# Cyame/glpk.js

Hardware: AMD Instinct MI355X
Metric: simplex pivots/s (dual, C3 dense 4096x16384 fp64) (higher is better)
Workload: dtype f64; 1 GPU; C3 dense random LP m=4096 n=16384 (BASELINE.json configs[2]); step = glp_simplex dual with it_lim=100 continuing from the previous basis; m=4096, n=16384, parallelism=replicas x1

## Files before the change

### glpk.js_amd/csrc/gk_dual.hip

```cpp
#include "gk_device.h"
#include <hip/hip_ext.h>
#include <algorithm>
#include <cstdlib>
#include <stdexcept>

namespace gk {

template <int NRHS, typename XF>
__device__ __forceinline__ void lgemv_tile(const double *__restrict__ M, size_t ld, int rows,
                                           const int *__restrict__ list, int t0, int t1, int r, XF xf,
                                           double *__restrict__ o)
{
    if (r >= rows) return;
    double a0 = 0.0, a1 = 0.0, b0 = 0.0, b1 = 0.0;
    int t = t0;
    for (; t + 4 <= t1; t += 4) {
        int c[4];
        double xa[4], xb[4];
        bool any = false;
#pragma unroll
        for (int u = 0; u < 4; ++u) {
            c[u] = list[t + u];
            xf(t + u, c[u], xa[u], xb[u]);
            any = any || xa[u] != 0.0 || xb[u] != 0.0;
// ... 185 lines not shown
    if (t < 0.0) t = 0.0;
    if (!(t <= tmax)) return false;
    e.k1 = t; e.k2 = fabs(alfa); e.idx = j + 1; e.aux = k;
    return true;
}

__device__ __forceinline__ Cand pass1_slot(const SpxDev &d, const RatioCtx &x, int idx)
{
    const int m = d.m, n = d.n;
    Cand best = no_cand(DBL_MAX);
    if (idx < n) {
        const int pos = d.bind[m + idx];
        if (pos > m) {
            const int j = pos - m - 1;
            Cand e;
            if (pass1_cand(x, d.trow[j], d.cbar[j], d.stat[j], j, m + idx + 1, e) && better<1>(e, best)) best = e;
        }
    }
    if (idx < m) {
        const int pos = d.bind[idx];
        if (pos > m) {
            const int j = pos - m - 1;
            Cand e;
            if (pass1_cand(x, d.trow[j], d.cbar[j], d.stat[j], j, idx + 1, e) && better<1>(e, best)) best = e;
        }
    }
    return best;
}

struct TopState {
    int iter_left, refact, refct;
    double obj;
};

struct FinishIn {
    int pend, p, q, kp, kq, fxp, rclr, upd_cnt, it_cnt, npiv, rig;
    double delta;
    TopState t;
};

__device__ __forceinline__ FinishIn finish_load(const SpxDev &d)
{
    const DState *st = d.st;
    FinishIn f;
    const int pend = st->pend, iter_left = st->iter_left, rpend = st->refact_pending, upd_cnt = st->upd_cnt,
              upd_lim = st->upd_lim, pricing = st->pricing, refct = st->refct, phase = st->phase;
    const double obj = st->obj, cqo = st->cbar_q_old, zeta = st->zeta, delta = st->delta, pivot = st->pivot;
    f.p = st->p; f.q = st->q; f.kp = st->kp; f.kq = st->kq;
    f.fxp = st->fxp; f.rclr = st->rclr; f.it_cnt = st->it_cnt; f.npiv = st->npiv;
    f.rig = st->rigorous;
    f.pend = pend;
    f.upd_cnt = upd_cnt;
    f.delta = delta;
    f.t.iter_left = iter_left - pend;
    f.t.refact = (rpend != 0) | ((pend != 0) & (upd_cnt + 1 >= upd_lim));
    f.t.refct = ((pend != 0) & (pricing == PT_PSE) & (refct > 0)) ? refct - 1 : refct;
    const double dobj = (cqo / zeta) * (delta / pivot);
    f.t.obj = ((pend != 0) & (phase == 2)) ? obj + dobj : obj;
    return f;
}

__device__ TopState finish_apply(const SpxDev &d, const FinishIn &f, bool tail_sync)
{
    DState *st = d.st;
    const int m = d.m;
    __syncthreads();
// ... 12 lines not shown
            st->binv_fresh = 0;
            st->cbar_fresh = 0;
            st->refact_pending = f.t.refact;
            st->it_cnt = f.it_cnt + 1;
            st->npiv = f.npiv + 1;
            st->iter_left = f.t.iter_left;
            if (f.rig > 0) st->rigorous = f.rig - 1;
            st->refct = f.t.refct;
            st->pend = 0;
        }
    }
    if (tail_sync) __syncthreads();
    return f.t;
}

__device__ __forceinline__ void finish_arrays(const SpxDev &d, const FinishIn &f)
{
    const int m = d.m;
    __syncthreads();
    if (f.pend) {
        if (threadIdx.x == 0) {
            d.head[f.p - 1] = f.kq;
            d.head[m + f.q - 1] = f.kp;
            d.bind[f.kq - 1] = f.p;
            d.bind[f.kp - 1] = m + f.q;
            d.stat[f.q - 1] = f.fxp ? NS : (f.delta > 0.0 ? NL : NU);
        } else if (threadIdx.x == 64) {
            if (f.rclr) d.refsp[f.kp - 1] = 0;
        }
    }
    __syncthreads();
}

__device__ __forceinline__ void finish_scalars(const SpxDev &d, const FinishIn &f, bool refsp_reset)
{
    DState *st = d.st;
    if (f.pend) {
        st->obj = f.t.obj;
        st->upd_cnt = f.upd_cnt + 1;
        st->binv_fresh = 0;
        st->cbar_fresh = 0;
        st->refact_pending = f.t.refact;
        st->it_cnt = f.it_cnt + 1;
        st->npiv = f.npiv + 1;
        st->iter_left = f.t.iter_left;
        if (f.rig > 0) st->rigorous = f.rig - 1;
        st->refct = f.t.refct;
        st->pend = 0;
    }
    if (refsp_reset) st->refct = 1000;
}

__device__ TopState dual_finish_block(const SpxDev &d, bool tail_sync)
{
    return finish_apply(d, finish_load(d), tail_sync);
}

__global__ void k_dual_finish(SpxDev d)
{
    (void)dual_finish_block(d, true);
}

__device__ __forceinline__ Cand chuzr_cand_v(int i, int k, int t, double lb, double ub, double bb, double g,
                                             double tol_bnd)
{
    double ri = 0.0;
// ... 82 lines not shown
    const double zeta = st->zeta, obj_ll = st->obj_ll, obj_ul = st->obj_ul;
    if (stop) return;
    const TopState ts = finish_apply(d, fin, false);
    if (ts.iter_left <= 0 || ts.refact) {
        if (threadIdx.x == 0) st->stop = ts.refact ? ST_REFACT : ST_BATCH;
        return;
    }
    if (pricing == PT_PSE && ts.refct == 0) {
        __syncthreads();
        reset_refsp_dev(d, 1);
        for (int l = threadIdx.x; l < n; l += blockDim.x) d.wpos[l] = -1;
        if (threadIdx.x == 0) st->nwl = 0;
        __syncthreads();
    }
    if (phase == 1) {
        if (!dinf) {
            if (threadIdx.x == 0) st->stop = ST_PHASE;
            return;
        }
    } else {
        const double z = zeta, obj = ts.obj;
        const bool hit = (z < 0.0 && obj_ll > -DBL_MAX && obj <= obj_ll) ||
                         (z > 0.0 && obj_ul < +DBL_MAX && obj >= obj_ul);
        if (hit) {
            if (threadIdx.x == 0) st->stop = ST_OBJLIM;
            return;
        }
    }
    const Cand best = wave_best<0>(c);
    if (best.idx == 0) {
        if (threadIdx.x == 0) { st->p = 0; st->stop = ST_P0; }
        return;
    }
    const int p = best.idx, kp = best.aux;
    if (rowpath == 3) {
        if (threadIdx.x == 0) {
            st->p = p;
            st->kp = kp;
            st->delta = best.k2;
            st->trow_max_bits = 0ull;
            st->ns = 0;
            st->dinf = 0;
        }
        return;
    }
    if (!rowpath) {
        for (int l = threadIdx.x; l < m; l += blockDim.x) d.rho[l] = 0.0;
        __syncthreads();
    }
    const double *brow = d.Binv + (p - 1);
    const size_t ldb = (size_t)d.ldb;
    double v[RPT];
#pragma unroll
    for (int u = 0; u < RPT; ++u) {
        const int t = threadIdx.x + u * TOP_WG;
        v[u] = (t < nr) ? brow[(size_t)cl[u] * ldb] : 0.0;
    }
#pragma unroll
    for (int u = 0; u < RPT; ++u) {
        const int t = threadIdx.x + u * TOP_WG;
        if (t < nr) {
            if (!rowpath) d.rho[cl[u]] = v[u];
            d.rho_idx[t] = cl[u];
            d.rho_val[t] = v[u];
        }
    }
    for (int t = threadIdx.x + RPT * TOP_WG; t < nr; t += blockDim.x) {
        const int cc = d.rlist[t];
        const double vv = brow[(size_t)cc * ldb];
        if (!rowpath) d.rho[cc] = vv;
        d.rho_idx[t] = cc;
        d.rho_val[t] = vv;
    }
    if (threadIdx.x == 0) {
        int ns = nr;
        if (kp <= m) {
            if (!rowpath) d.rho[kp - 1] = 1.0;
            d.rho_idx[nr] = kp - 1;
            d.rho_val[nr] = 1.0;
            ns++;
        }
        st->p = p;
        st->kp = kp;
        st->delta = best.k2;
        st->trow_max_bits = 0ull;
        st->ns = ns;
        st->dinf = 0;
    }
}

template <int PANEL>
__global__ void __launch_bounds__(256) k_dual_top_grid(SpxDev d, int pcap, int page_max)
{
    const TraceScope trace_(d, 0);
    DState *st = d.st;
    const int m = d.m, n = d.n;
    const int lane = threadIdx.x & 63;
    const bool lead = (blockIdx.x == 0);
    const int stop = st->stop;
    const FinishIn fin = finish_load(d);
    const int pricing = st->pricing, phase = st->phase, dinf = st->dinf, nr = st->nr;
    const double zeta = st->zeta, obj_ll = st->obj_ll, obj_ul = st->obj_ul;
    const int gm = 4 * ((m + 255) / 256);
    Cand cc = no_cand(0.0);
    for (int b = lane; b < gm; b += 64) {
        const Cand e = cand_chuzr(d)[b];
        if (better<0>(e, cc)) cc = e;
    }
    const int i = blockIdx.x * 256 + threadIdx.x;
    const int rp = (i < m) ? d.rpos[i] : -1;
    const int cl = (i < nr) ? d.rlist[i] : 0;
    if (stop) return;
    const TopState ts = fin.t;
    int why = ST_RUN;
    if (ts.iter_left <= 0 || ts.refact) why = ts.refact ? ST_REFACT : ST_BATCH;
    else if (phase == 1 && !dinf) why = ST_PHASE;
    else if (phase != 1 && ((zeta < 0.0 && obj_ll > -DBL_MAX && ts.obj <= obj_ll) ||
                            (zeta > 0.0 && obj_ul < +DBL_MAX && ts.obj >= obj_ul)))
        why = ST_OBJLIM;
    const Cand best = wave_best<0>(cc);
    if (why == ST_RUN && best.idx == 0) why = ST_P0;
    gate_arrive(st);
    if (why != ST_RUN) {
        if (lead) {
            if (threadIdx.x == 0) gate_wait(st);
            finish_arrays(d, fin);
            if (threadIdx.x == 0) {
                finish_scalars(d, fin, false);
                if (why == ST_P0) st->p = 0;
                st->stop = why;
            }
        }
        return;
    }
    const bool reset = pricing == PT_PSE && ts.refct == 0;
    if (lead) {
        if (threadIdx.x == 0) gate_wait(st);
        finish_arrays(d, fin);
        if (reset) {
            reset_refsp_dev(d, 1, false);
            for (int l = threadIdx.x; l < n; l += blockDim.x) d.wpos[l] = -1;
            if (threadIdx.x == 0) st->nwl = 0;
        }
        if (threadIdx.x == 0) finish_scalars(d, fin, reset);
    }
    const int p = best.idx, kp = best.aux;
    const double *brow = d.Binv + (p - 1);
    const size_t ldb = (size_t)d.ldb;
    const double vr = (i < m && rp >= 0) ? brow[(size_t)i * ldb] : 0.0;
    const double vl = (i < nr) ? brow[(size_t)cl * ldb] : 0.0;
    if (i < m) d.rho[i] = (rp >= 0) ? vr : (i == kp - 1 ? 1.0 : 0.0);
    if (i < nr) {
        d.rho_idx[i] = cl;
        d.rho_val[i] = vl;
// ... 218 lines not shown
    int c0[NP];
#pragma unroll
    for (int u = 0; u < NP; ++u) c0[u] = d.rlist[min(w + u * nw, m - 1)];
    int pos1 = d.bind[m + min(idx, n - 1)];
    int pos2 = d.bind[min(idx, m - 1)];
    const double *__restrict__ col = d.A.AT + min(idx, n - 1);
    const size_t ldt = (size_t)d.A.ldt;
    double a0[NP];
#pragma unroll
    for (int u = 0; u < NP; ++u) a0[u] = col[(size_t)min(max(c0[u], 0), m - 1) * ldt];
    Cand cc = no_cand(0.0);
#pragma unroll
    for (int u = 0; u < 4; ++u)
        if (lane + 64 * u < gm && better<0>(ce[u], cc)) cc = ce[u];
    for (int b = lane + 256; b < gm; b += 64) {
        const Cand e = cand_chuzr(d)[b];
        if (better<0>(e, cc)) cc = e;
    }
#pragma unroll
    for (int u = 0; u < NP; ++u) c0[u] = (w + u * nw < nr_cap) ? c0[u] : 0;
    if (w != 0 || idx >= n) pos1 = 0;
    if (w != 0 || idx >= m) pos2 = 0;
    if (stop) return;
    if (d.tslots && lead && threadIdx.x == 0) st->tk_start = wall_clock64();
    const TopState ts = fin.t;
    int why = ST_RUN;
    if (ts.iter_left <= 0 || ts.refact) why = ts.refact ? ST_REFACT : ST_BATCH;
    else if (phase == 1 && !dinf) why = ST_PHASE;
    else if (phase != 1 && ((zeta < 0.0 && obj_ll > -DBL_MAX && ts.obj <= obj_ll) ||
                            (zeta > 0.0 && obj_ul < +DBL_MAX && ts.obj >= obj_ul)))
        why = ST_OBJLIM;
    const Cand best = wave_best<0>(cc);
    if (why == ST_RUN && best.idx == 0) why = ST_P0;
    const bool reset = (why == ST_RUN && pricing == PT_PSE && ts.refct == 0);
    if (why != ST_RUN) {
        gate_arrive(st);
        if (lead) {
            if (threadIdx.x == 0) gate_wait(st);
            finish_arrays(d, fin);
            if (threadIdx.x == 0) {
                finish_scalars(d, fin, false);
                if (why == ST_P0) st->p = 0;
                st->stop = why;
            }
        }
        return;
    }
    if (lead) {
        finish_arrays(d, fin);
        if (reset) {
            reset_refsp_dev(d, 1, false);
            for (int l = threadIdx.x; l < n; l += blockDim.x) d.wpos[l] = -1;
            if (threadIdx.x == 0) st->nwl = 0;
        }
    }
    const int p = best.idx, kp = best.aux;
    const int ns = nr + (kp <= m ? 1 : 0);
    auto bind_new = [&](int k1, int v) {
        if (!fin.pend) return v;
        if (k1 == fin.kq) return fin.p;
        if (k1 == fin.kp) return m + fin.q;
        return v;
    };
    if (w == 0 && idx < n) pos1 = bind_new(m + idx + 1, pos1);
    if (w == 0 && idx < m) pos2 = bind_new(idx + 1, pos2);
    const int j1 = (pos1 > m) ? pos1 - m - 1 : -1;
    const int j2 = (pos2 > m) ? pos2 - m - 1 : -1;
    const double *__restrict__ brow = d.Binv + (p - 1);
    const size_t ldb = (size_t)d.ldb;
    double v0[NP];
#pragma unroll
    for (int u = 0; u < NP; ++u) {
        const int t = w + u * nw;
        int c = c0[u];
        double av = a0[u];
        if (t == nr) {
            c = kp - 1;
            av = col[(size_t)min(max(c, 0), m - 1) * ldt];
        }
        const int ca = min(max(c, 0), m - 1);
        const double bv = brow[(size_t)ca * ldb];
        v0[u] = (t < nr) ? bv : 1.0;
        a0[u] = (t < ns) ? av : 0.0;
        c0[u] = c;
    }
    const signed char stq = fin.fxp ? NS : (fin.delta > 0.0 ? NL : NU);
    int s1 = 0, s2 = 0;
    double cb1 = 0.0, cb2 = 0.0, rho2 = 0.0;
    bool ref1 = false, ref2 = false;
    if (w == 0) {
        const int j1c = max(j1, 0), j2c = max(j2, 0);
        const int l1 = d.stat[j1c], l2 = d.stat[j2c];
        const double c1 = d.cbar[j1c], c2 = d.cbar[j2c];
        const double r2 = brow[(size_t)min(idx, m - 1) * ldb];
        const int f1 = d.refsp[m + min(idx, n - 1)], f2 = d.refsp[min(idx, m - 1)];
        if (j1 >= 0) {
            s1 = (fin.pend && j1 == fin.q - 1) ? stq : l1;
            cb1 = c1;
            if (pse && !reset) ref1 = f1 != 0 && !(fin.pend && fin.rclr && m + idx + 1 == fin.kp);
        }
        if (j2 >= 0) {
            s2 = (fin.pend && j2 == fin.q - 1) ? stq : l2;
            cb2 = c2;
            rho2 = r2;
            if (pse && !reset) ref2 = f2 != 0 && !(fin.pend && fin.rclr && idx + 1 == fin.kp);
        }
    }
    double acc = 0.0;
#pragma unroll
    for (int u = 0; u < NP; ++u)
        if (w + u * nw < ns) acc += v0[u] * a0[u];
    if (lead && lane == 0) {
#pragma unroll
        for (int u = 0; u < NP; ++u) {
            const int t = w + u * nw;
            if (t < ns) {
                d.rho_idx[t] = c0[u];
                d.rho_val[t] = v0[u];
            }
        }
    }
    TPH(1, 0);
    {
        int t = w + NP * nw;
        for (; t < ns; t += 4 * nw) {
            int c[4];
            double v[4], a[4];
#pragma unroll
            for (int u = 0; u < 4; ++u) {
                const int tt = t + u * nw;
                c[u] = (tt < nr) ? d.rlist[tt] : kp - 1;
            }
#pragma unroll
            for (int u = 0; u < 4; ++u) {
                const int tt = t + u * nw;
                v[u] = (tt < nr) ? brow[(size_t)c[u] * ldb] : 1.0;
                a[u] = (tt < ns) ? col[(size_t)c[u] * ldt] : 0.0;
            }
#pragma unroll
            for (int u = 0; u < 4; ++u)
// ... 85 lines not shown
    constexpr int CU = 8;
    int beg = 0, end = 0;
    if (idx < n) {
        beg = d.A.cptr[idx];
        end = d.A.cptr[idx + 1];
    }
    int ci[CU];
    double cv[CU];
#pragma unroll
    for (int u = 0; u < CU; ++u) {
        const bool ok = beg + u < end;
        ci[u] = ok ? d.A.cind[beg + u] : 0;
        cv[u] = ok ? d.A.cval[beg + u] : 0.0;
    }
    constexpr int PU = 4;
    const int tpub = blockIdx.x * blockDim.x + threadIdx.x, npub = gridDim.x * blockDim.x;
    int cpub[PU];
#pragma unroll
    for (int u = 0; u < PU; ++u) {
        const int t = tpub + u * npub;
        cpub[u] = (t < nr_cap) ? d.rlist[t] : 0;
    }
    if (stop) return;
    if (d.tslots && lead && threadIdx.x == 0) st->tk_start = wall_clock64();
    const TopState ts = fin.t;
    int why = ST_RUN;
    if (ts.iter_left <= 0 || ts.refact) why = ts.refact ? ST_REFACT : ST_BATCH;
    else if (phase == 1 && !dinf) why = ST_PHASE;
    else if (phase != 1 && ((zeta < 0.0 && obj_ll > -DBL_MAX && ts.obj <= obj_ll) ||
                            (zeta > 0.0 && obj_ul < +DBL_MAX && ts.obj >= obj_ul)))
        why = ST_OBJLIM;
    const Cand best = wave_best<0>(cc);
    if (why == ST_RUN && best.idx == 0) why = ST_P0;
    const bool reset = (why == ST_RUN && pricing == PT_PSE && ts.refct == 0);
    gate_arrive(st);
    if (why != ST_RUN) {
        if (lead) {
            if (threadIdx.x == 0) gate_wait(st);
            finish_arrays(d, fin);
            if (threadIdx.x == 0) {
                finish_scalars(d, fin, false);
                if (why == ST_P0) st->p = 0;
                st->stop = why;
            }
        }
        return;
    }
    if (lead) {
        finish_arrays(d, fin);
        if (reset) {
            reset_refsp_dev(d, 1, false);
            for (int l = threadIdx.x; l < n; l += blockDim.x) d.wpos[l] = -1;
            if (threadIdx.x == 0) st->nwl = 0;
        }
    }
    const int p = best.idx, kp = best.aux;
    const int ns = nr + (kp <= m ? 1 : 0);
    auto bind_new = [&](int k1, int v) {
        if (!fin.pend) return v;
        if (k1 == fin.kq) return fin.p;
        if (k1 == fin.kp) return m + fin.q;
        return v;
    };
    if (idx < n) pos1 = bind_new(m + idx + 1, pos1);
    if (idx < m) pos2 = bind_new(idx + 1, pos2);
    const int j1 = (pos1 > m) ? pos1 - m - 1 : -1;
// ... 176 lines not shown
    }
    if ((int)blockIdx.x >= gn) {
        const int b = blockIdx.x - gn;
        const int tile = b % tiles_m, split = b / tiles_m, splits = (gridDim.x - gn) / tiles_m;
        const int cnt = st->nwl;
        if (stop) return;
        const int lps = (cnt + splits - 1) / splits;
        const int t0 = split * lps, t1 = min(cnt, t0 + lps);
        const int r = (tile * 256 + threadIdx.x) * 2;
        const double *wc = d.wcol;
        lgemv_tile<1>(d.A.A, (size_t)d.A.lda, m, d.wlist, t0, t1, r,
                      [&](int, int c, double &xa, double &xb) { xa = wc[c]; xb = 0.0; },
                      d.awpart + (size_t)split * m);
        __shared__ int last;
        __threadfence();
        __syncthreads();
        if (threadIdx.x == 0) last = (atomicAdd(&d.awcnt[tile], 1) == splits - 1);
        __syncthreads();
        if (!last) return;
        __threadfence();
        for (int rr = r; rr < min(r + 2, m); ++rr) {
            double acc = 0.0;
            for (int sp = 0; sp < splits; ++sp) acc += d.awpart[(size_t)sp * m + rr];
            d.work[rr] = d.ys[rr] - acc;
        }
        if (threadIdx.x == 0) d.awcnt[tile] = 0;
        return;
    }
    const int lane = threadIdx.x & 63;
    const bool stamps = d.tslots != nullptr;
    const unsigned long long t_entry = (stamps && rowpath && blockIdx.x == 0 && threadIdx.x == 0) ? wall_clock64() : 0ull;
    RatioIn rin = ratio_in(st);
    if (rowpath == 1) rin.delta = st->ob_delta;
    const int j = blockIdx.x * blockDim.x + threadIdx.x;
    const int jc = min(j, n - 1);
    double trj = d.trow[jc], cbj = d.cbar[jc];
    int sj = d.stat[jc], kj = d.head[m + jc];
    const bool lead = (blockIdx.x == 0 && threadIdx.x < 64);
    constexpr int CPL = 8;
    const bool bsplit = ncb > CPL * 64;
    const int tb = bsplit ? (int)threadIdx.x : lane, tst = bsplit ? (int)blockDim.x : 64;
    Cand cl[CPL];
    double tv[CPL];
#pragma unroll
    for (int u = 0; u < CPL; ++u) {
        const int b = min(tb + u * tst, ncb - 1);
        cl[u] = cand_pass1(d)[b];
        tv[u] = tmax_part(d)[b];
    }
    unsigned long long e = 0, xp = 0, u0 = 0;
    double uticks = 0.0, un = 0.0;
    if (stamps && rowpath && lead) {
        u0 = st->tk_upd0;
        uticks = st->upd_ticks;
        un = st->upd_n;
        unsigned long long te[CPL], tx[4];
#pragma unroll
        for (int u = 0; u < CPL; ++u) te[u] = d.tslots[min(lane + u * 64, ncb - 1)];
#pragma unroll
        for (int u = 0; u < 4; ++u) tx[u] = d.xslots[min(lane + u * 64, max(nprev - 1, 0))];
#pragma unroll
        for (int u = 0; u < CPL; ++u) e = max(e, te[u]);
#pragma unroll
        for (int u = 0; u < 4; ++u) xp = max(xp, tx[u]);
        for (int b = lane + CPL * 64; b < ncb; b += 64) e = max(e, d.tslots[b]);
        for (int b = lane + 4 * 64; b < nprev; b += 64) xp = max(xp, d.xslots[b]);
    }
    if (j >= n) { trj = 0.0; cbj = 0.0; sj = 0; kj = 0; }
    double v = 0.0;
#pragma unroll
    for (int u = 0; u < CPL; ++u) {
        if (tb + u * tst >= ncb) cl[u] = no_cand(DBL_MAX);
        else v = fmax(v, tv[u]);
    }
    for (int b = tb + CPL * tst; b < ncb; b += tst) v = fmax(v, tmax_part(d)[b]);
    double big = wmax(v);
    if (stop) return;
    __shared__ double rbig[4];
    __shared__ Cand rc1[4];
    __shared__ int rfl[4];
    if (bsplit) {
        if (lane == 0) rbig[threadIdx.x >> 6] = big;
        __syncthreads();
        big = fmax(fmax(rbig[0], rbig[1]), fmax(rbig[2], rbig[3]));
    }
    if (rowpath == 1 && blockIdx.x == 0 && threadIdx.x == 0) {
        const FinishIn f = finish_load(d);
        const int ob_p = st->ob_p, ob_kp = st->ob_kp, ob_ns = st->ob_ns, ob_reset = st->ob_reset;
        const double ob_delta = st->ob_delta;
        finish_scalars(d, f, ob_reset != 0);
        st->p = ob_p;
        st->kp = ob_kp;
        st->delta = ob_delta;
        st->ns = ob_ns;
        st->dinf = 0;
    }
    TPH(2, 0);
    if (lead) {
        const unsigned long long ee = stamps ? wmax_u64(e) : 0ull, xx = stamps ? wmax_u64(xp) : 0ull;
        if (lane == 0) {
            st->trow_max_bits = dbits(big);
            if (stamps && rowpath) {
                st->tk_next = t_entry;
                st->tk_end = ee;
                st->tk_prev = xx;
                if (u0 != 0ull && xx > u0 && xx - u0 < 20000ull) {
                    st->upd_ticks = uticks + (double)(xx - u0);
                    st->upd_n = un + 1.0;
                }
                st->tk_upd0 = 0ull;
            }
        }
    }
    const RatioCtx x = ratio_ctx(rin, big);
    Cand c = no_cand(DBL_MAX);
    int fail = 0;
#pragma unroll
    for (int u = 0; u < CPL; ++u) {
        if (cl[u].idx != 0 && cl[u].k2 < x.eps) fail = 1;
        else if (better<1>(cl[u], c)) c = cl[u];
    }
    for (int b = tb + CPL * tst; b < ncb; b += tst) {
        const Cand f = cand_pass1(d)[b];
        if (f.idx != 0 && f.k2 < x.eps) fail = 1;
        else if (better<1>(f, c)) c = f;
    }
// ... 777 lines not shown
    }
    const int rc = min(r, m - 1);
    const int kold_l = d.head[rc];
    double bb = d.bbar[rc];
    double g = (NRHS == 2) ? d.gamma[rc] : 0.0;
    const int JPB = (n + gridDim.x - 1) / gridDim.x;
    const int j = blockIdx.x * JPB + (int)threadIdx.x;
    const bool colth = (int)threadIdx.x < JPB && j < n;
    const int jc = min(j, n - 1);
    double cb = d.cbar[jc];
    double tri = d.trow[jc];
    int hkj = d.head[m + jc];
    pin.c = no_cand(0.0);
#pragma unroll
    for (int u = 0; u < 4; ++u)
        if (lane + 64 * u < np2 && better<2>(c2l[u], pin.c)) pin.c = c2l[u];
    for (int b = lane + 256; b < np2; b += 64) {
        const Cand e = cand_pass2(d)[b];
        if (better<2>(e, pin.c)) pin.c = e;
    }
    pin.g = 0.0;
    if (NRHS == 2 && w == 0) {
#pragma unroll
        for (int u = 0; u < 4; ++u)
            if (lane + 64 * u < ncb) pin.g += gp[u];
        for (int b = lane + 256; b < ncb; b += 64) pin.g += d.gpart[b];
    }
#pragma unroll
    for (int u = 0; u < GM; ++u)
        if (gs + u * NSL > nr_cap) { c0[u] = 0; rv[u] = 0.0; }
    const int kold = rowlane ? kold_l : 1;
    if (!rowlane) { bb = 0.0; g = 0.0; }
    if (!colth) { cb = 0.0; tri = 0.0; hkj = 1; }
    TPH(3, 0);
    const double gsum = (NRHS == 2 && w == 0) ? wsum(pin.g) : 0.0;
    const PickOut pk = pick_choose(pin);
    const int q = pk.q, kq = pk.kq;
    const int qc = min(max(q, 1), n), kqc = min(max(kq, 1), m + n);
    const bool hdense = !SP && kqc > m;
    const double *__restrict__ hcolv = d.A.A + (size_t)(hdense ? kqc - m - 1 : 0) * d.A.lda;
    double bv[GM], xa[GM], xb[GM];
#pragma unroll
    for (int u = 0; u < GM; ++u) {
        const int ca = min(max(c0[u], 0), m - 1);
        bv[u] = Bv[(size_t)ca * ldb + rc];
        xa[u] = SP ? 0.0 : hcolv[ca];
        xb[u] = (NRHS == 2) ? d.work[ca] : 0.0;
    }
    const int kou = min(max(kold - 1, 0), m - 1);
    const double ua_l = SP ? 0.0 : hcolv[kou];
    const double ub_l = (NRHS == 2) ? d.work[kou] : 0.0;
    const int tkp = d.type[kp - 1];
    const bool refkp = NRHS == 2 && d.refsp[kp - 1] != 0;
    const int knew = (r == p - 1) ? kqc : kold;
    const int tkold_l = d.type[kold - 1];
    const int refk_l = (NRHS == 2) ? d.refsp[kold - 1] : 0;
    const int tknew_l = d.type[knew - 1];
    const double lbn_l = d.lb[knew - 1], ubn_l = d.ub[knew - 1];
    const int stq_l = d.stat[qc - 1];
    const double lbq = d.lb[kqc - 1], ubq = d.ub[kqc - 1];
    const int tkq = d.type[kqc - 1];
    const double piv2 = d.trow[qc - 1];
    const int kn = colth ? ((j == q - 1) ? kp : hkj) : 1;
    const int ot_l = d.orig_type[kn - 1];
    if (bk && w == wa) {
        Books b;
        books_load<NRHS>(d, b, nr, kqc);
        if (lane == 0) sbk = b;
    }
    if (stop) return;
    const bool lead = bk && threadIdx.x == 0;
    if (q == 0) {
        if (lead) { st->q = 0; st->stop = ST_Q0; }
        return;
    }
    if (pk.alfa < 1e-5 * (1.0 + 0.01 * pin.big) && !pin.rigorous) {
        if (lead) { st->q = q; st->stop = ST_SMALLPIV; }
        return;
// ... 465 lines not shown
        return;
    }
    if (pl.colpath) {
        if (ev0) (void)hipEventRecord(ev0, s);
        hipLaunchKernelGGL(k_dual_col, dim3(gv), dim3(256), 0, s, d, pl.pse, pl.nr_cap, pl.gm);
        if (ev1) (void)hipEventRecord(ev1, s);
        hipLaunchKernelGGL(k_dual_ratio, dim3(gn + (pl.pse ? cdiv(m, 256) + d.A.nlr : 0)), dim3(256), 0, s, d, gn,
                           tiles_m, 2, ncb, 0, prev_blocks(d, pl));
        if (pl.fupd) {
            if (pl.pse) launch_update<2, 1>(s, d, pl, gn, ncb, 2);
            else launch_update<1, 1>(s, d, pl, gn, ncb, 2);
            return;
        }
        if (pl.pse)
            hipLaunchKernelGGL((k_dual_ftran1<2, 1, 16>), dim3(cdiv(m, 16)), dim3(64 * pl.fwaves), 0, s, d, gn,
                               pl.awsplits, ncb, pl.nr_cap);
        else
            hipLaunchKernelGGL((k_dual_ftran1<1, 1, 16>), dim3(cdiv(m, 16)), dim3(64 * pl.fwaves), 0, s, d, gn,
                               pl.awsplits, ncb, pl.nr_cap);
        hipLaunchKernelGGL(k_dual_commit, dim3(gv + tiles_m * pl.uchunks), dim3(256), 0, s, d, pl.pse, gv, tiles_m,
                           pl.lpsu, 2, bytes_fixed(d), 0);
        return;
    }
    if (pl.rowpath) {
        ncb = cdiv(std::max(m, n), 64);
        if (ev0)
            hipExtLaunchKernelGGL(k_dual_row<8>, dim3(ncb), dim3(64 * pl.twaves), 0, s, ev0, ev1, 0, d, pl.pse,
                                  pl.nr_cap, pl.gm);
        else
            hipLaunchKernelGGL(k_dual_row<8>, dim3(ncb), dim3(64 * pl.twaves), 0, s, d, pl.pse, pl.nr_cap, pl.gm);
    } else {
        const bool tgrid = !pl.rigorous && d.A.dense && m >= 1024;
        if (tgrid && pl.panel)
            hipLaunchKernelGGL(k_dual_top_grid<1>, dim3(cdiv(m, 256)), dim3(256), 0, s, d, pl.panel, pl.panel_age);
        else if (tgrid)
            hipLaunchKernelGGL(k_dual_top_grid<0>, dim3(cdiv(m, 256)), dim3(256), 0, s, d, 0, pl.panel_age);
        else
            hipLaunchKernelGGL(k_dual_top, dim3(1), dim3(TOP_WG), 0, s, d, pl.rowpath, pl.nr_cap);
        if (pl.rigorous) refine_rho_dev(s, d);
        if (ev0) (void)hipEventRecord(ev0, s);
        if (pl.panel)
            panel_trow(s, d, pl, tgrid);
        else if (d.shard && d.shard->vsize > 1)
            lp_shard_sim(s, d, pl.pse);
        else if (d.shard) {
            const LpShard &sh = *d.shard;
            const int lo = std::min(n, sh.rank * sh.L), hi = std::min(n, lo + sh.L);
            colpass_gated(s, d.A, CP_TROW, m + lo, hi - lo, d.head, d.stat + lo, d.coef, nullptr, d.rho, nullptr,
                          d.trow + lo, nullptr, &d.st->trow_max_bits, d.st, 0);
            lp_shard_trow(s, d, pl.pse);
        } else
            colpass_gated(s, d.A, CP_TROW, m, n, d.head, d.stat, d.coef, nullptr, d.rho, nullptr, d.trow, nullptr,
                          nullptr, d.st, 0);
        if (ev1) (void)hipEventRecord(ev1, s);
        hipLaunchKernelGGL(k_trow_finish, dim3(gv), dim3(256), 0, s, d, pl.pse, (pl.panel ? 1 : 0) | (d.shard ? 2 : 0));
    }
    const int aw = (pl.pse && d.A.dense && !d.shard) ? 1 : 0;
    const int awone = (aw && pl.fused) ? pl.awone : 0;
    hipLaunchKernelGGL(k_dual_ratio, dim3(gn + (aw ? (awone ? cdiv(m, 64) : tiles_m * pl.awsplits) : 0)), dim3(256), 0,
                       s, d, gn, tiles_m, pl.rowpath, ncb, awone, prev_blocks(d, pl));
    if (pl.fupd) {
        if (pl.pse) launch_update<2, 0>(s, d, pl, gn, ncb, pl.rowpath, ev2, ev3);
        else launch_update<1, 0>(s, d, pl, gn, ncb, pl.rowpath, ev2, ev3);
        return;
    }
    if (pl.fused) {
        if (pl.fone) {
            if (pl.pse)
                hipLaunchKernelGGL((k_dual_ftran1<2, 0, 64>), dim3(cdiv(m, 64)), dim3(64 * pl.fwaves), 0, s, d, gn,
// ... 216 lines not shown
```

### glpk.js_amd/csrc/gk_engine.hip

```cpp
#include "gk_device.h"
#include "../../include/glpk_mi355x.h"

#include <algorithm>
#include <chrono>
#include <cfloat>
#include <cmath>
#include <cstdarg>
#include <cstdio>
#include <cstring>
#include <string>
#include <type_traits>
#include <vector>

using namespace gk;

namespace {

thread_local std::string g_err;

void set_err(const char *fmt, ...)
{
    char buf[1024];
    va_list ap;
    va_start(ap, fmt);
// ... 1976 lines not shown
    mark("batch");
    const double t0 = now_s();
    const int k_chain0 = hs.upd_cnt;
    struct T { gk_bfd *f; double t0; ~T() { f->stats.seconds_batches += now_s() - t0; } } tt{f, t0};
    epi_drop();
    bool armed = false;
    hs.stop = ST_RUN;
    std::memset(hs.gate, 0, sizeof hs.gate);
    hs.iter_left = K;
    hs.npiv = 0;
    hs.phase = phase;
    hs.rigorous = rigorous;
    hs.dinf = 0;
    hs.pend = 0;
    push_state();
    if (dual && E->dense && (E->pnl_m != m || E->pnl_n != n)) {
        const int ldp = (n + 7) & ~7;
        E->pnl.ensure((size_t)PANEL_MAX * ldp);
        E->pnl_src.ensure((size_t)PANEL_MAX * m);
        E->pslot.ensure(m);
        E->ppos.ensure(PANEL_MAX);
        HIPCHK(hipMemsetAsync(E->pslot.p, 0xff, (size_t)m * sizeof(int), s));
        HIPCHK(hipMemsetAsync(E->ppos.p, 0, PANEL_MAX * sizeof(int), s));
        E->pnl_m = m;
        E->pnl_n = n;
    }
    SpxDev d = dev();
    const int pse = (parm->pricing == PT_PSE);
    if (dual) {
        auto bucket = [](int x, int cap) {
            int g = std::max(64, x / 8);
            return std::min(cap, (x + g - 1) / g * g);
        };
        DualPlan pl = dual_plan(d, bucket(hs.nr + K + 1, m), bucket(hs.nwl + K + 1, n), pse, rigorous);
        pl.sparse = f->sparse ? 1 : 0;
        const int evp = E->prof == 1 || E->prof == 2;
        if (evp) prof_events(K);
        const bool shard_eager = d.shard && d.shard->vsize <= 1 && gk_comm_backend(d.shard->comm) != GK_COMM_RCCL;
        if (d.shard) d.shard->exchanges += K;
        static const bool no_graph = [] {
            const char *e = std::getenv("GK_NO_GRAPH");
            return e && std::atoi(e) != 0;
        }();
        if (!rigorous && K >= 4 && !evp && !f->sparse && !shard_eager && !no_graph) {
            run_graph(d, pl, K);
            armed = epi_arm(K);
        } else {
            dual_batch_begin(s, d, pl);
            for (int t = 0; t < K; t++) dual_iteration2(s, d, pl, ev0(t), ev1(t), ev2(t), ev3(t));
            dual_batch_end(s, d, pl);
            ev_upd = evp && pl.fupd && pl.rowpath;
        }
    } else if (f->sparse) {
        primal_batch_begin(s, d);
        for (int t = 0; t < K; t++) primal_iteration_sparse(s, d, pse);
    } else if (!rigorous && primal_fast_ok(d)) {
        if (lists_stale) {
            rebuild_lists();
            d = dev();
        }
        auto bucket = [](int x, int cap) {
            int g = std::max(64, x / 8);
            return std::min(cap, (x + g - 1) / g * g);
        };
        const DualPlan pl = primal_plan(d, bucket(hs.nr + K + 1, m), pse);
        if (K >= 4) run_graph(d, pl, K, 1);
        else {
// ... 115 lines not shown
            break;
        }
    if (!hit) {
        hipGraph_t graph = nullptr;
        HIPCHK(hipStreamBeginCapture(s, hipStreamCaptureModeThreadLocal));
        if (kind == 0) {
            if (part != 2) dual_batch_begin(s, d, pl);
            for (int t = 0; t < K; t++) dual_iteration2(s, d, pl);
            if (part != 1) dual_batch_end(s, d, pl);
        } else {
            if (part != 2) primal_batch_begin(s, d);
            for (int t = 0; t < K; t++) primal_iteration2(s, d, pl);
        }
        HIPCHK(hipStreamEndCapture(s, &graph));
        hipGraphExec_t exec = nullptr;
        HIPCHK(hipGraphInstantiate(&exec, graph, nullptr, nullptr, 0));
        (void)hipGraphDestroy(graph);
        if (En.graphs.size() >= 24) {
            auto lru = std::min_element(En.graphs.begin(), En.graphs.end(),
                                        [](const GraphEntry &a, const GraphEntry &b) { return a.last < b.last; });
            (void)hipGraphExecDestroy(lru->exec);
            En.graphs.erase(lru);
        }
        GraphEntry g;
        g.d = d; g.pl = pl; g.K = K; g.kind = key; g.exec = exec;
        En.graphs.push_back(g);
        hit = &En.graphs.back();
        f->stats.graphs_built++;
    }
    hit->last = ++En.graph_clock;
    HIPCHK(hipGraphLaunch(hit->exec, s));
}

static int next_batch(int k, int why) { return why == ST_BATCH ? std::min(2 * k, 64) : 8; }

static int align_to_refactor(int K, int left)
{
    if (left <= 0 || left >= K) return K;
    if (left < 8) return left;
    int p = 8;
    while (2 * p <= left) p *= 2;
    return p;
}

int Spx::run_dual()
{
    const gk_smcp *P = parm;
    int binv_st = f->valid ? 2 : 0, bbar_st = 0, cbar_st = 0, rigorous = 0;
    int ret;
    for (;;) {
        if (binv_st == 0) {
            pull();
            drift_arm(cbar, cbar_st);
            const long long nref0 = f->stats.refinements;
            if (!reinvert()) {
                report_msg(GK_MSG_FACTERR, 1, fact_ret);
                return fail_return();
            }
            det_log(f->stats.refinements != nref0 ? "reinv-newton" : "reinv");
            binv_st = 1;
            bbar_st = cbar_st = 0;
            hs.upd_cnt = sp_replayed; hs.refact_pending = 0; hs.grow_bits = 0;
        }
        hs.binv_fresh = (binv_st == 1);
        int feas_pre = -1;
        if (cbar_st == 0) {
            dinf_known = false;
// ... 126 lines not shown
                return it_hit ? 8 : 9;
            }
        }
        if (hs.refact_pending && binv_st != 0) {
            binv_st = 0;
            refine_next = (hs.echk == echk_seen);
            continue;
        }
        display(0);
        int K = rigorous ? 1 : E->kbatch;
        if (P->it_lim < 0x7fffffff) {
            const int rem = P->it_lim - (hs.it_cnt - it_beg);
            K = (!rigorous && K >= 64 && rem <= 128) ? rem : std::max(1, std::min(K, rem));
        }
        K = align_to_refactor(K, hs.upd_lim - hs.upd_cnt);
        K = ahead_align(K);
        K = align_to_display(K);
        int why = batch(K, rigorous);
        if (f->sparse) ahead_maybe();
        det_log("batch", K, why);
        if (f->sparse) sp_stamps_dump(*f->sp, s, ctx->wall_khz);
        E->kbatch = next_batch(E->kbatch, why);
        dinf_known = (why == ST_BATCH && hs.npiv > 0);
        if (hs.npiv > 0) {
            bbar_st = 2;
            cbar_st = 2;
            binv_st = 2;
            rigorous = hs.rigorous;
        }
        switch (why) {
        case ST_BATCH:
        case ST_PHASE:
        case ST_OBJLIM:
            break;
        case ST_REFACT:
            binv_st = 0;
            refine_next = (hs.echk == echk_seen);
            break;
        case ST_P0:
            if (bbar_st != 1 || cbar_st != 1) {
                if (bbar_st != 1) bbar_st = 0;
                if (cbar_st != 1) cbar_st = 0;
                break;
            }
            {
                display(1);
                report_msg(phase == 1 ? GK_MSG_NODFS : GK_MSG_OPTIMAL, 3);
                int p_stat, d_stat;
                if (phase == 1) {
                    pull();
                    set_orig_bnds();
                    eval_bbar();
                    p_stat = 3; d_stat = 4;
                } else
                    p_stat = d_stat = 2;
                store_sol(p_stat, d_stat, 0);
            }
            return 0;
        case ST_Q0:
            if (bbar_st != 1 || cbar_st != 1 || !rigorous) {
                if (bbar_st != 1) bbar_st = 0;
                if (cbar_st != 1) cbar_st = 0;
                rigorous = 1;
                break;
            }
            display(1);
// ... 867 lines not shown
```

### glpk.js_amd/csrc/gk_internal.h

```cpp
#pragma once
#include <hip/hip_runtime.h>
#include <cstdint>
#include <cstddef>
#include <vector>

struct gk_comm;

namespace gk {

enum : int {
    FR = 1, LO = 2, UP = 3, DB = 4, FX = 5,
    BS = 1, NL = 2, NU = 3, NF = 4, NS = 5,
    PT_STD = 0x11, PT_PSE = 0x22, RT_STD = 0x11, RT_HAR = 0x22,
};

enum : int {
    ST_RUN = 0,
    ST_BATCH = 1,
    ST_PHASE = 2,
    ST_OBJLIM = 3,
    ST_P0 = 4,
    ST_Q0 = 5,
    ST_SMALLPIV = 6,
    ST_PIVCHK = 7,
    ST_DCHK = 8,
    ST_REFACT = 9,
    ST_REFSP = 10,
};
constexpr int EPI_GATE = 0x100;


struct DState {
    int stop, p, q, p_stat;
    int phase, it_cnt, npiv, iter_left;
    int refct, upd_cnt, upd_lim, rigorous;
    int binv_fresh, cbar_fresh, pricing, rtest;
    int refact_pending, nr, ns, nw;
    int ce, pend, dinf, nwl;
    int need2, q1, pad0, pad1;
    double delta, teta, new_dq, cbar_q_new;
    double gamma_pq, eta_pq, pivot, xnq;
    double zeta, tol_bnd, tol_dj, tol_piv;
    double obj_ll, obj_ul, obj, tcol_max;
    double cbar_q_old, bytes;
    double teta1, bytes_trow;
    unsigned long long tk_start, tk_end;
    unsigned long long tk_next, tk_pad;
    double trow_ticks, trow_n;
    double trow_ticks_b, trow_pad;
    unsigned long long trow_max_bits, tcol_max_bits;
    int kp, kq, fxp, rclr;
    int kq1, echk, page, pad4;
    double alfa1;
    unsigned long long grow_bits;
    unsigned long long tk_prev, tk_pad2;
    double trow_ticks_r, trow_nr;
    unsigned long long tk_upd0, tk_pad3;
    double upd_ticks, upd_n;
    double bytes_upd, upd_tol;
    int pk, pcur, pmiss, pvalid;
    double phits, pmisses;
// ... 221 lines not shown
```

Measured before the change: 12470 pivots/s.

## Cap planned row-list size with slack and stop batch early when full

The planned nonzero-row capacity (nr_cap) is now sized from the current count plus a configurable slack instead of the worst-case growth over the whole batch. When the list would overflow, a new stop reason ST_CAP ends the batch early without halving the next batch size. Smaller capacities are meant to shrink the per-pivot kernels' work and register footprint, at the cost of more frequent batch restarts. Smaller tweaks move the non-reset finish_arrays onto a single thread to skip block barriers, hoist the outbox finish loads and the Binv loads earlier to hide latency, and clamp nr_cap to a threshold of 254 when possible.

```diff
diff --git a/glpk.js_amd/csrc/gk_dual.hip b/glpk.js_amd/csrc/gk_dual.hip
--- a/glpk.js_amd/csrc/gk_dual.hip
+++ b/glpk.js_amd/csrc/gk_dual.hip
@@ -241,6 +241,8 @@
     int iter_left, refact, refct;
     double obj;
 };
+
+__device__ __forceinline__ bool list_full(int nr, int nr_cap, int m) { return nr + 1 > nr_cap && nr_cap < m; }
 
 struct FinishIn {
     int pend, p, q, kp, kq, fxp, rclr, upd_cnt, it_cnt, npiv, rig;
@@ -319,6 +321,19 @@
     __syncthreads();
 }
 
+__device__ __forceinline__ void finish_arrays_wave0(const SpxDev &d, const FinishIn &f)
+{
+    const int m = d.m;
+    if (f.pend) {
+        d.head[f.p - 1] = f.kq;
+        d.head[m + f.q - 1] = f.kp;
+        d.bind[f.kq - 1] = f.p;
+        d.bind[f.kp - 1] = m + f.q;
+        d.stat[f.q - 1] = f.fxp ? NS : (f.delta > 0.0 ? NL : NU);
+        if (f.rclr) d.refsp[f.kp - 1] = 0;
+    }
+}
+
 __device__ __forceinline__ void finish_scalars(const SpxDev &d, const FinishIn &f, bool refsp_reset)
 {
     DState *st = d.st;
@@ -467,6 +482,10 @@
         if (threadIdx.x == 0) { st->p = 0; st->stop = ST_P0; }
         return;
     }
+    if (rowpath != 3 && list_full(nr, nr_cap, m)) {
+        if (threadIdx.x == 0) st->stop = ST_CAP;
+        return;
+    }
     const int p = best.idx, kp = best.aux;
     if (rowpath == 3) {
         if (threadIdx.x == 0) {
@@ -525,7 +544,7 @@
 }
 
 template <int PANEL>
-__global__ void __launch_bounds__(256) k_dual_top_grid(SpxDev d, int pcap, int page_max)
+__global__ void __launch_bounds__(256) k_dual_top_grid(SpxDev d, int pcap, int page_max, int nr_cap)
 {
     const TraceScope trace_(d, 0);
     DState *st = d.st;
@@ -555,6 +574,7 @@
         why = ST_OBJLIM;
     const Cand best = wave_best<0>(cc);
     if (why == ST_RUN && best.idx == 0) why = ST_P0;
+    if (why == ST_RUN && list_full(nr, nr_cap, m)) why = ST_CAP;
     gate_arrive(st);
     if (why != ST_RUN) {
         if (lead) {
@@ -839,6 +859,7 @@
         why = ST_OBJLIM;
     const Cand best = wave_best<0>(cc);
     if (why == ST_RUN && best.idx == 0) why = ST_P0;
+    if (why == ST_RUN && list_full(nr, nr_cap, m)) why = ST_CAP;
     const bool reset = (why == ST_RUN && pricing == PT_PSE && ts.refct == 0);
     if (why != ST_RUN) {
         gate_arrive(st);
@@ -853,13 +874,11 @@
         }
         return;
     }
-    if (lead) {
+    if (lead && reset) {
         finish_arrays(d, fin);
-        if (reset) {
-            reset_refsp_dev(d, 1, false);
-            for (int l = threadIdx.x; l < n; l += blockDim.x) d.wpos[l] = -1;
-            if (threadIdx.x == 0) st->nwl = 0;
-        }
+        reset_refsp_dev(d, 1, false);
+        for (int l = threadIdx.x; l < n; l += blockDim.x) d.wpos[l] = -1;
+        if (threadIdx.x == 0) st->nwl = 0;
     }
     const int p = best.idx, kp = best.aux;
     const int ns = nr + (kp <= m ? 1 : 0);
@@ -913,6 +932,7 @@
             if (pse && !reset) ref2 = f2 != 0 && !(fin.pend && fin.rclr && idx + 1 == fin.kp);
         }
     }
+    if (lead && !reset && threadIdx.x == 0) finish_arrays_wave0(d, fin);
     double acc = 0.0;
 #pragma unroll
     for (int u = 0; u < NP; ++u)
@@ -1064,6 +1084,7 @@
         why = ST_OBJLIM;
     const Cand best = wave_best<0>(cc);
     if (why == ST_RUN && best.idx == 0) why = ST_P0;
+    if (why == ST_RUN && list_full(nr, nr_cap, m)) why = ST_CAP;
     const bool reset = (why == ST_RUN && pricing == PT_PSE && ts.refct == 0);
     gate_arrive(st);
     if (why != ST_RUN) {
@@ -1306,6 +1327,13 @@
     const unsigned long long t_entry = (stamps && rowpath && blockIdx.x == 0 && threadIdx.x == 0) ? wall_clock64() : 0ull;
     RatioIn rin = ratio_in(st);
     if (rowpath == 1) rin.delta = st->ob_delta;
+    const bool outbox = rowpath == 1 && blockIdx.x == 0 && threadIdx.x < 64;
+    FinishIn obf = {};
+    int ob_p = 0, ob_kp = 0, ob_ns = 0, ob_reset = 0;
+    if (outbox) {
+        obf = finish_load(d);
+        ob_p = st->ob_p; ob_kp = st->ob_kp; ob_ns = st->ob_ns; ob_reset = st->ob_reset;
+    }
     const int j = blockIdx.x * blockDim.x + threadIdx.x;
     const int jc = min(j, n - 1);
     double trj = d.trow[jc], cbj = d.cbar[jc];
@@ -1358,14 +1386,11 @@
         __syncthreads();
         big = fmax(fmax(rbig[0], rbig[1]), fmax(rbig[2], rbig[3]));
     }
-    if (rowpath == 1 && blockIdx.x == 0 && threadIdx.x == 0) {
-        const FinishIn f = finish_load(d);
-        const int ob_p = st->ob_p, ob_kp = st->ob_kp, ob_ns = st->ob_ns, ob_reset = st->ob_reset;
-        const double ob_delta = st->ob_delta;
-        finish_scalars(d, f, ob_reset != 0);
+    if (outbox && threadIdx.x == 0) {
+        finish_scalars(d, obf, ob_reset != 0);
         st->p = ob_p;
         st->kp = ob_kp;
-        st->delta = ob_delta;
+        st->delta = rin.delta;
         st->ns = ob_ns;
         st->dinf = 0;
     }
@@ -2209,6 +2234,9 @@
     const int kold = rowlane ? kold_l : 1;
     if (!rowlane) { bb = 0.0; g = 0.0; }
     if (!colth) { cb = 0.0; tri = 0.0; hkj = 1; }
+    double bv[GM];
+#pragma unroll
+    for (int u = 0; u < GM; ++u) bv[u] = Bv[(size_t)min(max(c0[u], 0), m - 1) * ldb + rc];
     TPH(3, 0);
     const double gsum = (NRHS == 2 && w == 0) ? wsum(pin.g) : 0.0;
     const PickOut pk = pick_choose(pin);
@@ -2216,11 +2244,10 @@
     const int qc = min(max(q, 1), n), kqc = min(max(kq, 1), m + n);
     const bool hdense = !SP && kqc > m;
     const double *__restrict__ hcolv = d.A.A + (size_t)(hdense ? kqc - m - 1 : 0) * d.A.lda;
-    double bv[GM], xa[GM], xb[GM];
+    double xa[GM], xb[GM];
 #pragma unroll
     for (int u = 0; u < GM; ++u) {
         const int ca = min(max(c0[u], 0), m - 1);
-        bv[u] = Bv[(size_t)ca * ldb + rc];
         xa[u] = SP ? 0.0 : hcolv[ca];
         xb[u] = (NRHS == 2) ? d.work[ca] : 0.0;
     }
@@ -2752,9 +2779,10 @@
     } else {
         const bool tgrid = !pl.rigorous && d.A.dense && m >= 1024;
         if (tgrid && pl.panel)
-            hipLaunchKernelGGL(k_dual_top_grid<1>, dim3(cdiv(m, 256)), dim3(256), 0, s, d, pl.panel, pl.panel_age);
+            hipLaunchKernelGGL(k_dual_top_grid<1>, dim3(cdiv(m, 256)), dim3(256), 0, s, d, pl.panel, pl.panel_age,
+                               pl.nr_cap);
         else if (tgrid)
-            hipLaunchKernelGGL(k_dual_top_grid<0>, dim3(cdiv(m, 256)), dim3(256), 0, s, d, 0, pl.panel_age);
+            hipLaunchKernelGGL(k_dual_top_grid<0>, dim3(cdiv(m, 256)), dim3(256), 0, s, d, 0, pl.panel_age, pl.nr_cap);
         else
             hipLaunchKernelGGL(k_dual_top, dim3(1), dim3(TOP_WG), 0, s, d, pl.rowpath, pl.nr_cap);
         if (pl.rigorous) refine_rho_dev(s, d);
diff --git a/glpk.js_amd/csrc/gk_engine.hip b/glpk.js_amd/csrc/gk_engine.hip
--- a/glpk.js_amd/csrc/gk_engine.hip
+++ b/glpk.js_amd/csrc/gk_engine.hip
@@ -2032,7 +2032,11 @@
             int g = std::max(64, x / 8);
             return std::min(cap, (x + g - 1) / g * g);
         };
-        DualPlan pl = dual_plan(d, bucket(hs.nr + K + 1, m), bucket(hs.nwl + K + 1, n), pse, rigorous);
+        const char *es = std::getenv("GK_PLAN_SLACK");
+        const int slack = std::max(1, es ? std::atoi(es) : 32);
+        int nr_cap = std::min(bucket(hs.nr + slack, m), bucket(hs.nr + K + 1, m));
+        if (nr_cap > DUAL_UPDATE_NR_MAX && hs.nr + slack <= DUAL_UPDATE_NR_MAX) nr_cap = DUAL_UPDATE_NR_MAX;
+        DualPlan pl = dual_plan(d, nr_cap, bucket(hs.nwl + K + 1, n), pse, rigorous);
         pl.sparse = f->sparse ? 1 : 0;
         const int evp = E->prof == 1 || E->prof == 2;
         if (evp) prof_events(K);
@@ -2214,7 +2218,7 @@
     HIPCHK(hipGraphLaunch(hit->exec, s));
 }
 
-static int next_batch(int k, int why) { return why == ST_BATCH ? std::min(2 * k, 64) : 8; }
+static int next_batch(int k, int why) { return why == ST_BATCH ? std::min(2 * k, 64) : (why == ST_CAP ? k : 8); }
 
 static int align_to_refactor(int K, int left)
 {
@@ -2407,6 +2411,7 @@
         case ST_BATCH:
         case ST_PHASE:
         case ST_OBJLIM:
+        case ST_CAP:
             break;
         case ST_REFACT:
             binv_st = 0;
diff --git a/glpk.js_amd/csrc/gk_internal.h b/glpk.js_amd/csrc/gk_internal.h
--- a/glpk.js_amd/csrc/gk_internal.h
+++ b/glpk.js_amd/csrc/gk_internal.h
@@ -26,7 +26,9 @@
     ST_DCHK = 8,
     ST_REFACT = 9,
     ST_REFSP = 10,
-};
+    ST_CAP = 11,
+};
+constexpr int DUAL_UPDATE_NR_MAX = 254;
 constexpr int EPI_GATE = 0x100;
 
 
```

After: 12660 pivots/s, median of 6. 1.02x the previous value.
